# foxcroftjn/polars-strsim

Measured on AMD Instinct MI355X. Metric: M string-pairs/s, levenshtein, 100 M rows (+ achieved HBM GB/s in roofline), higher is better.
Workload: dtype u8/u32 bit-parallel, f64 epilogue

## Files before the change

polars-strsim_amd/csrc/strsim_kernels.hip:

```cpp
#include <hip/hip_runtime.h>
#include <stddef.h>
#include <cstdlib>
#include <stdint.h>
#include <type_traits>

#include "strsim_bounds.h"
#include "strsim_lane_core.h"
#include "strsim_lane_lut.h"
#include "strsim_lane_wide.h"
#include "strsim_lane_sym.h"
#include "strsim_kernels.h"
#include "strsim_lane_common.h"
#include "strsim_osa.h"
#include "strsim_distance.h"
#include "strsim_indel.h"
#include "strsim_partial.h"
#include "strsim_qgram.h"
#include "strsim_token.h"
#include "strsim_wratio.h"
#include "strsim_process.h"
#include "strsim_nearest.h"
#include "strsim_extract.h"
#include "strsim_cdist.h"
#include "strsim_join.h"
#include "strsim_match_join.h"
#include "strsim_components.h"

namespace strsim {

constexpr int ALL_MEASURES = 5;

struct OutPtrs {
    double *p[5];
};

#include "strsim_lane_stage.h"
#if defined(STRSIM_LAB) && defined(STRSIM_STAGE_PC)
#include "strsim_lane_stage_pc.h"
#endif
#include "strsim_lane_lit.h"
#include "strsim_match.h"
#include "strsim_nearest_kernels.h"
#include "strsim_extract_kernels.h"
#include "strsim_cdist_kernels.h"
#include "strsim_join_kernels.h"
#include "strsim_match_join_kernels.h"
#include "strsim_components_kernels.h"

#include "strsim_kernel_wide.h"
#include "strsim_kernel_utf8.h"
#include "strsim_kernel_wave.h"
#include "strsim_kernel_huge.h"

static void wide_geometry(const LaunchArgs &a, int span, uint32_t &sps, unsigned &grid)
{
    const uint64_t nchunks = (a.n + 63u) >> 6;
    const uint64_t nspans = (nchunks + (uint64_t)span - 1) / (uint64_t)span;
    const uint64_t want = 2u * (uint64_t)a.wide_grid;
    uint64_t k = nspans / (want ? want : 1u);
    if (k < 1u) k = 1u;
    if (k > (uint64_t)(WIDE_BLOCK / span)) k = WIDE_BLOCK / span;
    sps = (uint32_t)k;
    const uint64_t nsuper = (nspans + k - 1u) / k;
    grid = (unsigned)(nsuper < (uint64_t)a.wide_grid_cap ? nsuper : (uint64_t)a.wide_grid_cap);
}

static uint64_t stage_launch_size(uint64_t nsb, uint64_t resident, uint64_t cus)
{
    constexpr uint64_t per = 4;
    uint64_t g = nsb / per;
    const uint64_t floor_ = nsb < cus ? nsb : cus;
    if (g < floor_) g = floor_;
    if (g > resident) g = resident;
    return g ? g : 1u;
}

template <int M>
static void launch_lane_t(const LaunchArgs &a)
{
#if defined(STRSIM_LAB) && defined(STRSIM_STAGE_STRIP)
    if (M == LEVENSHTEIN && a.rowsA != 1 && a.rowsB != 1) {
        static uint16_t *buf = nullptr;
        static uint64_t cap = 0;
        if (a.n > cap) { if (buf) (void)hipFree(buf); (void)hipMalloc((void **)&buf, a.n * 2 + 64); cap = a.n; }
        hipLaunchKernelGGL(k_strip_oracle, dim3((unsigned)((a.n + 255) / 256)), dim3(256), 0, a.stream, a.offA, a.valA, a.offB, a.valB, a.n, buf);
        (void)hipMemcpyToSymbolAsync(HIP_SYMBOL(g_strip_ptr), &buf, sizeof buf, 0, hipMemcpyHostToDevice, a.stream);
    }
#endif
    if (a.ev_lane0) (void)hipEventRecord(a.ev_lane0, a.stream);
    OutPtrs op{};
    op.p[0] = a.out;
    const bool lit_a = a.rowsA == 1 && a.rowsB != 1, lit_b = a.rowsB == 1 && a.rowsA != 1;
    const bool lit_path = lit_a || lit_b;
    if (lit_path && !a.no_literal_path) {
        const bool litA = lit_a;
        const uint64_t nlb = (a.n + (LIT_ROWS - 1)) / LIT_ROWS;
        const uint64_t want = (uint64_t)a.stage_grid * 3u;
        const uint64_t gl = nlb < want ? nlb : want;
        hipLaunchKernelGGL((k_lane_lit<M>), dim3((unsigned)gl), dim3(LIT_BLOCK), 0, a.stream, litA ? a.offB : a.offA,
                           litA ? a.valB : a.valA, litA ? a.offA : a.offB, litA ? a.valA : a.valB, a.out, a.n, a.slowmask,
                           a.status, a.qtab, a.sched);
        if (a.publish_host) hipLaunchKernelGGL(k_publish_lit, dim3(1), dim3(64), 0, a.stream, a.sched, a.publish_host, a.publish_ticket);
    } else {
        const uint64_t nsb = (a.n + (STAGE_ROWS - 1)) / STAGE_ROWS;
        auto go = [&](auto tables, auto long_rows) {
            constexpr bool T = decltype(tables)::value, L = decltype(long_rows)::value;
            const uint64_t res = (uint64_t)a.stage_grid * (uint64_t)stage_waves_per_eu<M, T, L>() / (uint64_t)STRSIM_STAGE_WAVES_PER_EU;
            const uint64_t gs = stage_launch_size(nsb, res, (uint64_t)a.stage_grid / (uint64_t)STRSIM_STAGE_WAVES_PER_EU);
            hipLaunchKernelGGL((k_lane_stage<M, T, L>), dim3((unsigned)gs), dim3(STAGE_BLOCK), 0, a.stream, a.offA, a.valA, a.rowsA,
                               a.offB, a.valB, a.rowsB, op, a.n, a.slowmask, a.status, a.qtab, a.sched, a.publish_host, a.publish_ticket);
        };
#if defined(STRSIM_LAB) && defined(STRSIM_STAGE_PC)
        if (((STRSIM_STAGE_PC >> M) & 1) != 0 && a.rowsA != 1 && a.rowsB != 1 && !a.long_rows) {
            const uint64_t cus = (uint64_t)a.stage_grid / (uint64_t)STRSIM_STAGE_WAVES_PER_EU;
            const uint64_t gs = stage_launch_size(nsb, cus * (uint64_t)STRSIM_PC_WG_PER_CU, cus);
            hipLaunchKernelGGL((k_lane_stage_pc<M, STRSIM_PC_LUT != 0>), dim3((unsigned)gs), dim3(PC_THREADS), 0, a.stream, a.offA, a.valA, a.rowsA,
                               a.offB, a.valB, a.rowsB, op, a.n, a.slowmask, a.status, a.qtab, a.sched, a.publish_host, a.publish_ticket);
        } else
#endif
        if (a.long_rows) go(std::false_type{}, std::true_type{});
        else if constexpr (stage_uses_lut<M>()) go(std::true_type{}, std::false_type{});
        else go(std::false_type{}, std::false_type{});
    }
    if (a.ev_lane1) (void)hipEventRecord(a.ev_lane1, a.stream);
}

template <int M>
static void launch_slow_t(const LaunchArgs &a)
{
    const uint64_t nchunks = (a.n + 63u) >> 6;
    const uint64_t wg = M == LEVENSHTEIN ? (uint64_t)a.wave_grid_lev
                        : (M == JARO || M == JARO_WINKLER) ? (uint64_t)a.wave_grid * 3u / 4u : (uint64_t)a.wave_grid;
    const uint64_t g2 = nchunks < wg ? nchunks : wg;
    {
        uint32_t sps, sps8;
        unsigned g3, g8;
        wide_geometry(a, WIDE_SPAN, sps, g3);
        wide_geometry(a, U8_SPAN, sps8, g8);
        hipLaunchKernelGGL((k_lane_wide<M>), dim3(g3), dim3(WIDE_BLOCK), 0, a.stream, a.offA, a.valA, a.rowsA,
                           a.offB, a.valB, a.rowsB, a.out, a.n, a.slowmask, sps);
        hipLaunchKernelGGL((k_lane_utf8<M>), dim3(g8), dim3(WIDE_BLOCK), 0, a.stream, a.offA, a.valA, a.rowsA,
                           a.offB, a.valB, a.rowsB, a.out, a.n, a.slowmask, sps8, a.worklist, a.status);
    }
    hipLaunchKernelGGL((k_wave_pairs<M>), dim3((unsigned)g2), dim3(64), 0, a.stream, a.offA, a.valA, a.rowsA, a.offB,
                       a.valB, a.rowsB, a.out, a.n, a.slowmask, a.worklist, a.status, a.lev_ws);
    if (a.ev_wave1) (void)hipEventRecord(a.ev_wave1, a.stream);
}


template <int M>
static void launch_pair(const LaunchArgs &a)
{
    launch_lane_t<M>(a);
    launch_slow_t<M>(a);
}

template <int M>
static void launch_huge_t(const LaunchArgs &a, uint32_t *ws, uint32_t cap, int grid)
{
    hipLaunchKernelGGL((k_huge_pairs<M>), dim3((unsigned)grid), dim3(64), 0, a.stream, a.offA, a.valA, a.rowsA, a.offB,
                       a.valB, a.rowsB, a.out, a.n, ws, cap);
// ... 702 lines not shown
```

polars-strsim_amd/csrc/strsim_lane_stage.h:

```cpp
#pragma once

#ifndef STRSIM_STAGE_ROWS
#define STRSIM_STAGE_ROWS 512
#endif
#ifndef STRSIM_STAGE_CAP
#define STRSIM_STAGE_CAP 10240
#endif
#ifndef STRSIM_STAGE_CAP_LONG
#define STRSIM_STAGE_CAP_LONG 15104
#endif
#ifndef STRSIM_STAGE_CAP_LUT
#define STRSIM_STAGE_CAP_LUT 8960
#endif
#ifndef STRSIM_STAGE_WAVES_PER_EU
#define STRSIM_STAGE_WAVES_PER_EU 5
#endif
#ifndef STRSIM_STAGE_BUCKET_SHIFT
#define STRSIM_STAGE_BUCKET_SHIFT 1
#endif

#ifndef STRSIM_STAGE_LUT
#define STRSIM_STAGE_LUT 0x26
#endif
#ifndef STRSIM_JARO_KEEP_EQ_FILLS
#define STRSIM_JARO_KEEP_EQ_FILLS 1
#endif
#ifndef STRSIM_STAGE_LONG_TEXT_MAX
#define STRSIM_STAGE_LONG_TEXT_MAX 32
#endif
#ifndef STRSIM_STAGE_RANGE_MAX
#define STRSIM_STAGE_RANGE_MAX 64
#endif
#ifndef STRSIM_STAGE_RANGE_DIV
#define STRSIM_STAGE_RANGE_DIV 4
#endif
#ifndef STRSIM_STAGE_RANGE_MIN_BLOCKS
#define STRSIM_STAGE_RANGE_MIN_BLOCKS 2
#endif

#if defined(STRSIM_LAB) && defined(STRSIM_STAGE_STAMPS)
__device__ unsigned long long g_stage_stamps[16384][16];
#define STAGE_STAMP(cat) do { __builtin_amdgcn_sched_barrier(0); const unsigned long long t_ = __builtin_amdgcn_s_memtime(); \
                              __builtin_amdgcn_sched_barrier(0); st_acc[cat] += t_ - st_last; st_last = t_; } while (0)
#else
#define STAGE_STAMP(cat) do { } while (0)
#endif

#ifndef STRSIM_STAGE_THREADS
#define STRSIM_STAGE_THREADS 256
#endif
constexpr int STAGE_BLOCK = STRSIM_STAGE_THREADS;
constexpr int STAGE_WAVES = STAGE_BLOCK / 64;
constexpr int STAGE_ROWS = STRSIM_STAGE_ROWS;
constexpr int STAGE_RPT = STAGE_ROWS / STAGE_BLOCK;
constexpr int STAGE_NR = STAGE_ROWS / 64;
constexpr int STAGE_RPW = STAGE_NR / STAGE_WAVES;
template <int MEASURE> constexpr bool stage_uses_lut() { return ((STRSIM_STAGE_LUT >> MEASURE) & 1) != 0; }

template <bool TABLES, bool LONG = false> struct StageGeom {
    static_assert(!(TABLES && LONG), "the long-row geometry has no match-mask tables");
    static constexpr int CAP = LONG ? STRSIM_STAGE_CAP_LONG : (TABLES ? STRSIM_STAGE_CAP_LUT : STRSIM_STAGE_CAP);
    static constexpr int COL = CAP + 96;
    static constexpr int DMA_ITERS = (CAP + 48 + 16 * STAGE_BLOCK - 1) / (16 * STAGE_BLOCK);
    static_assert(CAP % 16 == 0 && 2 * COL + 64 + 16 <= 65536, "staging area: whole wave-instructions, 16-bit LDS offsets");
};
constexpr int STAGE_BSH = STRSIM_STAGE_BUCKET_SHIFT;
constexpr int STAGE_NBK = (32 >> STAGE_BSH) + 1;
static_assert(STAGE_RPT >= 1 && STAGE_RPT <= 4 && STAGE_RPW >= 1, "STAGE_ROWS is 256, 512 or 1024");
static_assert(STAGE_NBK <= 32, "the bucket scan runs on 32 lanes");

#define STRSIM_LDS_ADDR(p) ((uint32_t)(uintptr_t)((__attribute__((address_space(3))) void *)(p)))

__device__ __forceinline__ void lds_dma_b128(const void *gbase, uint32_t goff, uint32_t lds_dst)
{
    uint32_t keep;
    asm volatile("s_mov_b32 %0, m0\n\ts_mov_b32 m0, %3\n\ts_nop 0\n\tglobal_load_lds_dwordx4 %1, %2\n\ts_mov_b32 m0, %0"
                 : "=&s"(keep)
                 : "v"(goff), "s"(gbase), "s"(lds_dst)
                 : "memory");
}
__device__ __forceinline__ void lds_dma_b32(const void *gbase, uint32_t goff, uint32_t lds_dst)
{
    uint32_t keep;
    asm volatile("s_mov_b32 %0, m0\n\ts_mov_b32 m0, %3\n\ts_nop 0\n\tglobal_load_lds_dword %1, %2\n\ts_mov_b32 m0, %0"
                 : "=&s"(keep)
                 : "v"(goff), "s"(gbase), "s"(lds_dst)
                 : "memory");
}

__device__ __forceinline__ uint32_t load_invariant(const uint32_t *p)
{
    return *reinterpret_cast<const __attribute__((address_space(4))) uint32_t *>(reinterpret_cast<uintptr_t>(p));
}

constexpr uint32_t STAGE_DEAD = 1u << 31;

#if defined(STRSIM_LAB) && defined(STRSIM_STAGE_STRIP)
__device__ const uint16_t *g_strip_ptr;
__global__ __launch_bounds__(256) void k_strip_oracle(const uint32_t *__restrict__ offA, const uint8_t *__restrict__ valA, const uint32_t *__restrict__ offB,
                                                      const uint8_t *__restrict__ valB, uint64_t n, uint16_t *__restrict__ out)
{
    const uint64_t r = (uint64_t)blockIdx.x * 256u + threadIdx.x;
    if (r >= n) return;
    const uint32_t a0 = offA[r], la = offA[r + 1] - a0, b0 = offB[r], lb = offB[r + 1] - b0;
    const uint32_t m = la < lb ? la : lb, cap = (uint32_t)STRSIM_STAGE_STRIP;
    uint32_t p = 0, s = 0;
    while (p < m && p < cap && valA[a0 + p] == valB[b0 + p]) ++p;
    while (s < m - p && s < cap && valA[a0 + la - 1u - s] == valB[b0 + lb - 1u - s]) ++s;
    if (p + s > 63u) s = 63u - p;
    out[r] = (uint16_t)(p | (s << 8));
}
#define STRSIM_STRIP_ON 1
#else
#define STRSIM_STRIP_ON 0
#endif

__device__ __forceinline__ void stage_window(const uint8_t *base, uint32_t at, uint32_t (&w)[8], uint32_t lds_bytes = 0u, uint32_t who = 0u)
{
    typedef uint32_t u32x4_a4 __attribute__((ext_vector_type(4), aligned(4)));
    (void)lds_bytes; (void)who;
    if (who == 1u) STRSIM_CHECK_RANGE(K_STAGE, 40, ~0ull, (at & ~3u) + 36u, 0, lds_bytes);
    if (who == 2u) STRSIM_CHECK_RANGE(K_LIT, 40, ~0ull, (at & ~3u) + 36u, 0, lds_bytes);
    const uint8_t *q = base + (at & ~3u);
    const u32x4_a4 lo = *reinterpret_cast<const u32x4_a4 *>(q);
    const u32x4_a4 hi = *reinterpret_cast<const u32x4_a4 *>(q + 16);
    const uint32_t top = *reinterpret_cast<const uint32_t *>(q + 32);
    const uint32_t sh = at & 3u;
    w[0] = __builtin_amdgcn_alignbyte(lo.y, lo.x, sh); w[1] = __builtin_amdgcn_alignbyte(lo.z, lo.y, sh);
    w[2] = __builtin_amdgcn_alignbyte(lo.w, lo.z, sh); w[3] = __builtin_amdgcn_alignbyte(hi.x, lo.w, sh);
    w[4] = __builtin_amdgcn_alignbyte(hi.y, hi.x, sh); w[5] = __builtin_amdgcn_alignbyte(hi.z, hi.y, sh);
    w[6] = __builtin_amdgcn_alignbyte(hi.w, hi.z, sh); w[7] = __builtin_amdgcn_alignbyte(top, hi.w, sh);
}

__device__ __forceinline__ uint32_t scan32_inclusive(uint32_t x)
{
    x += (uint32_t)__builtin_amdgcn_update_dpp(0, (int)x, 0x111, 0xF, 0xF, true);
    x += (uint32_t)__builtin_amdgcn_update_dpp(0, (int)x, 0x112, 0xF, 0xF, true);
    x += (uint32_t)__builtin_amdgcn_update_dpp(0, (int)x, 0x114, 0xF, 0xF, true);
    x += (uint32_t)__builtin_amdgcn_update_dpp(0, (int)x, 0x118, 0xF, 0xF, true);
    x += (uint32_t)__builtin_amdgcn_update_dpp(0, (int)x, 0x142, 0xA, 0xF, true);
    return x;
}

template <int NP, bool USE_LUT>
__device__ __forceinline__ uint32_t stage_lev_code(const EqLut &lut, const uint32_t (&wa)[8], uint32_t la, const uint32_t (&wb)[8],
                                                   uint32_t lb, uint32_t tmin, uint32_t tmax, uint32_t stripped = 0u)
{
    uint32_t P[NP];
    build_planes<NP>(wb, P);
    EqLut t = lut;
    if (USE_LUT) lut_build<NP>(t, P, 0xFFFFFFFFu);
    const bool live = la != 0u && lb != 0u;
    const uint32_t la1 = live ? la : 1u, lb1 = live ? lb : 1u;
    const uint32_t dist = USE_LUT ? lev_myers32_lut<NP>(t, wa, la1, tmin, tmax, P, lb1) : lev_myers32_snap<NP>(wa, la1, tmin, tmax, P, lb1);
    uint32_t code = dist * (uint32_t)QTAB_N + (la1 > lb1 ? la1 : lb1);
    if (!live) code = (la == 0u && lb == 0u) ? 1u : (uint32_t)QTAB_N + 1u;
#if STRSIM_STRIP_ON
    const uint32_t longer = la > lb ? la : lb;
    code = (live ? dist : longer) * (uint32_t)QTAB_N + (longer + stripped);
#endif
    return code;
}

template <int NP, bool USE_LUT>
__device__ __forceinline__ unsigned long long stage_all_ints(const EqLut &lut, const uint32_t (&wa)[8], uint32_t la,
                                                             const uint32_t (&wb)[8], uint32_t lb, uint32_t tmin, uint32_t tmax)
{
    uint32_t P[NP];
    build_planes<NP>(wb, P);
    const bool live = la != 0u && lb != 0u;
    const uint32_t la1 = live ? la : 1u, lb1 = live ? lb : 1u;
    uint32_t dist, m, t, isect;
    if (USE_LUT) {
        EqLut tb = lut;
        lut_build<NP>(tb, P, 0xFFFFFFFFu);
        lane_cores32_lut<NP, true, true, true>(tb, wa, la1, tmin, tmax, lb1, P, dist, m, t, isect);
    } else {
        lane_cores32<NP, true, true, true>(wa, la1, tmin, tmax, lb1, P, dist, m, t, isect);
    }
    const uint32_t pre = common_prefix4(wa[0], la1, wb[0], lb1);
    const uint32_t lo = dist | (m << 6) | (t << 12) | (isect << 18) | (pre << 24) | (la << 27);
    return (unsigned long long)lo | ((unsigned long long)(la >> 5) << 32) | ((unsigned long long)lb << 33);
}

__device__ __forceinline__ void stage_all_epilogues(unsigned long long pk, double qa, double qb, double qc, double qd, double (&r)[5])
{
    const uint32_t lo = (uint32_t)pk, hi = (uint32_t)(pk >> 32);
    const uint32_t m = (lo >> 6) & 63u, isect = (lo >> 18) & 63u, pre = (lo >> 24) & 7u;
    const uint32_t la = ((lo >> 27) & 31u) | ((hi & 1u) << 5), lb = (hi >> 1) & 63u;
    if (la == 0u || lb == 0u) {
        const double v = (la == 0u && lb == 0u) ? 1.0 : 0.0;
#pragma unroll
        for (int q = 0; q < 5; ++q) r[q] = v;
        return;
    }
    r[LEVENSHTEIN] = 1.0 - qd;
    const double j = m == 0u ? 0.0 : div3_exact(qa + qb + qc);
    r[JARO] = j;
    r[JARO_WINKLER] = epilogue_jaro_winkler(j, pre);
    r[JACCARD] = epilogue_jaccard(isect, la, lb);
    r[SORENSEN_DICE] = epilogue_sorensen_dice(isect, la, lb);
}

template <int MEASURE, int NP, bool USE_LUT>
__device__ __forceinline__ uint32_t stage_ints(const EqLut &lut, const uint32_t (&wa)[8], uint32_t la, const uint32_t (&wb)[8],
                                               uint32_t lb, uint32_t tmin, uint32_t tmax)
{
    uint32_t P[NP];
    build_planes<NP>(wb, P);
    const bool live = la != 0u && lb != 0u;
    const uint32_t la1 = live ? la : 1u, lb1 = live ? lb : 1u;
    uint32_t dist, m, t, isect;
    EqLut tb = lut;
    if (USE_LUT) lut_build<NP>(tb, P, 0xFFFFFFFFu);
    if (MEASURE == JARO || MEASURE == JARO_WINKLER) {
        if (USE_LUT) lane_cores32_lut<NP, false, true, false>(tb, wa, la1, tmin, tmax, lb1, P, dist, m, t, isect);
        else lane_cores32<NP, false, true, false, STRSIM_JARO_KEEP_EQ_FILLS != 0>(wa, la1, tmin, tmax, lb1, P, dist, m, t, isect);
        const uint32_t pre = MEASURE == JARO_WINKLER ? common_prefix4(wa[0], la1, wb[0], lb1) : 0u;
        return m | (t << 6) | (la << 12) | (lb << 18) | (pre << 24);
    }
    if (USE_LUT) lane_cores32_lut<NP, false, false, true>(tb, wa, la1, tmin, tmax, lb1, P, dist, m, t, isect);
    else lane_cores32<NP, false, false, true>(wa, la1, tmin, tmax, lb1, P, dist, m, t, isect);
    return isect | (la << 6) | (lb << 12);
}

template <int MEASURE>
__device__ __forceinline__ double stage_epilogue(uint32_t pk, double qa, double qb, double qc)
{
    if (MEASURE == JARO || MEASURE == JARO_WINKLER) {
        const uint32_t m = pk & 63u, la = (pk >> 12) & 63u, lb = (pk >> 18) & 63u, pre = (pk >> 24) & 7u;
        if (la == 0u || lb == 0u) return (la == 0u && lb == 0u) ? 1.0 : 0.0;
        const double j = m == 0u ? 0.0 : div3_exact(qa + qb + qc);
        return MEASURE == JARO_WINKLER ? epilogue_jaro_winkler(j, pre) : j;
    }
    const uint32_t isect = pk & 63u, la = (pk >> 6) & 63u, lb = (pk >> 12) & 63u;
    if (la == 0u || lb == 0u) return (la == 0u && lb == 0u) ? 1.0 : 0.0;
    return MEASURE == JACCARD ? epilogue_jaccard(isect, la, lb) : epilogue_sorensen_dice(isect, la, lb);
}

template <int MEASURE, bool LUT>
__device__ __forceinline__ void stage_compute(const EqLut &lut, const uint32_t (&wt)[8], const uint32_t (&wp)[8], uint32_t meta,
                                              uint32_t last, uint16_t *s_code, uint32_t *s_word, double *s_val)
{
    bool fast = (meta & STAGE_DEAD) == 0u;
#if STRSIM_STRIP_ON
    const uint32_t lt = meta & 0x3Fu, lp = (meta >> 8) & 0x3Fu, idx = (meta >> 16) & 0x1FFu, stripped = (meta >> 25) & 0x3Fu;
#else
    const uint32_t lt = meta & 0x3Fu, lp = (meta >> 8) & 0x3Fu, idx = (meta >> 16) & 0x7FFu, stripped = 0u;
#endif
    uint32_t any;
    const uint32_t vary = window_vary(wt, wp, any);
    if (any & 0x80u) fast = false;
    if (__ballot(fast) == 0ull) return;
    const uint32_t la = fast ? lt : 0u, lb = fast ? lp : 0u;
    static_assert((1 << STAGE_BSH) % COLS_PER_TEST == 0, "a bucket's upper bound is a whole number of column groups");
    const uint32_t ltl = (uint32_t)__builtin_amdgcn_readlane((int)lt, (int)last);
    const uint32_t tmax = (((ltl ? ltl : 1u) - 1u) | ((1u << STAGE_BSH) - 1u)) + 1u;
    const bool wide = __ballot(fast && (vary & 0x60u)) != 0ull;
    const uint32_t lt0 = uniform(lt);
    const uint32_t tmin = (((lt0 ? lt0 : 1u) - 1u) & ~((1u << STAGE_BSH) - 1u)) + 1u;
    if (MEASURE == LEVENSHTEIN) {
        uint32_t code;
        if (wide) code = stage_lev_code<7, LUT>(lut, wt, la, wp, lb, tmin, tmax, stripped);
        else code = stage_lev_code<5, LUT>(lut, wt, la, wp, lb, tmin, tmax, stripped);
        if (fast) STRSIM_CHECK_INDEX(K_STAGE, 42, ~0ull, idx, STAGE_ROWS);
        if (fast) s_code[idx] = (uint16_t)code;
    } else if (MEASURE == ALL_MEASURES) {
        unsigned long long pk;
        if (wide) pk = stage_all_ints<7, LUT>(lut, wt, la, wp, lb, tmin, tmax);
        else pk = stage_all_ints<5, LUT>(lut, wt, la, wp, lb, tmin, tmax);
        if (fast) STRSIM_CHECK_INDEX(K_STAGE, 43, ~0ull, idx, STAGE_ROWS);
        if (fast) reinterpret_cast<unsigned long long *>(s_val)[idx] = pk;
    } else {
        uint32_t pk;
        if (wide) pk = stage_ints<MEASURE, 7, LUT>(lut, wt, la, wp, lb, tmin, tmax);
        else pk = stage_ints<MEASURE, 5, LUT>(lut, wt, la, wp, lb, tmin, tmax);
        if (fast) STRSIM_CHECK_INDEX(K_STAGE, 44, ~0ull, idx, STAGE_ROWS);
        if (fast) s_word[idx] = pk;
    }
}

template <int MEASURE, bool LUT, bool LONG = false>
__device__ __forceinline__ void
lane_stage_body(const uint32_t *__restrict__ offA, const uint8_t *__restrict__ valA, uint64_t rowsA,
             const uint32_t *__restrict__ offB, const uint8_t *__restrict__ valB, uint64_t rowsB, OutPtrs outs,
             uint64_t n, unsigned long long *__restrict__ slowmask, DevStatus *__restrict__ status,
             const double *__restrict__ qtab, uint32_t *__restrict__ sched, DevStatus *__restrict__ publish, uint32_t ticket)
{
    constexpr bool LEV = MEASURE == LEVENSHTEIN;
    constexpr bool ALL = MEASURE == ALL_MEASURES;
    constexpr int B = STAGE_ROWS, RPT = STAGE_RPT, NBK = STAGE_NBK;
    constexpr int STAGE_CAP = StageGeom<LUT, LONG>::CAP, STAGE_COL = StageGeom<LUT, LONG>::COL;
    constexpr int STAGE_DMA_ITERS = StageGeom<LUT, LONG>::DMA_ITERS;
    constexpr uint32_t COLB = STAGE_COL, LIT = 2u * STAGE_COL;
    static_assert(!LUT || (B <= 128 * STAGE_WAVES && LUT_WAVE_BYTES == 3072), "descriptor slices: 128 rows behind each wave's tables");
    __shared__ __attribute__((aligned(4096))) uint8_t s_lut[LUT ? 4096 * STAGE_WAVES : 16];
    __shared__ uint2 s_desc_own[LUT ? 1 : B];
    __shared__ __attribute__((aligned(4096))) uint8_t s_bytes[2 * STAGE_COL + 64 + 16];
    auto desc_at = [&](uint32_t p) -> uint2 * {
        if (LUT) return reinterpret_cast<uint2 *>(s_lut + ((p >> 7) << 12) + LUT_WAVE_BYTES + ((p & 127u) << 3));
        return s_desc_own + p;
    };
    __shared__ __attribute__((aligned(16))) uint32_t s_off[2][B + 4];
    __shared__ uint32_t s_cnt[32];
    __shared__ uint32_t s_left;
    __shared__ uint32_t s_sched[2];
    __shared__ uint16_t s_code[LEV ? B : 1];
    __shared__ uint32_t s_word[(!LEV && !ALL) ? B : 1];
    __shared__ double s_val[ALL ? B : 1];

    const uint32_t tid = threadIdx.x, lane = lane_id(), wv = tid >> 6;
    if (blockIdx.x == 0u && tid < (uint32_t)(sizeof(DevStatus) / sizeof(uint32_t))) reinterpret_cast<uint32_t *>(status)[tid] = 0u;
    if (tid < 32u) s_cnt[tid] = 0u;
    if (tid == 0u) s_left = 0u;
#pragma unroll
    for (int q = 0; q < RPT; ++q) {
        const uint32_t i = (uint32_t)q * STAGE_BLOCK + tid;
        if (LEV) s_code[i] = 0xFFFFu;
        else if (ALL) reinterpret_cast<unsigned long long *>(&s_val[i])[0] = ~0ull;
        else s_word[i] = 0xFFFFFFFFu;
    }

    const uint32_t totalA = load_invariant(offA + rowsA), totalB = load_invariant(offB + rowsB);
#if STRSIM_BOUNDS_ON
    const uint32_t firstA = load_invariant(offA), firstB = load_invariant(offB);
#endif
    const bool bcastA = rowsA == 1, bcastB = rowsB == 1;
    const uint32_t litA0 = bcastA ? load_invariant(offA) : 0u, litB0 = bcastB ? load_invariant(offB) : 0u;
    const uint32_t litAlen = bcastA ? totalA - litA0 : 0u, litBlen = bcastB ? totalB - litB0 : 0u;
    if (wv == 0u) {
        auto literal_window = [&](const uint8_t *val, uint32_t at, uint32_t total, uint32_t len, uint32_t *dst) {
            uint32_t w[8];
            load_window32(val, at, total, w);
            const uint32_t rep = (w[0] & 0xFFu) * 0x01010101u;
#pragma unroll
            for (int q = 0; q < 8; ++q) {
                const uint32_t v = len > 4u * q ? (len - 4u * q < 4u ? len - 4u * q : 4u) : 0u;
                const uint32_t keep = v >= 4u ? 0xFFFFFFFFu : ((1u << (8u * v)) - 1u);
                dst[q] = (w[q] & keep) | (rep & ~keep);
            }
        };
        if (bcastA) literal_window(valA, litA0, totalA, litAlen, reinterpret_cast<uint32_t *>(s_bytes + LIT));
        if (bcastB) literal_window(valB, litB0, totalB, litBlen, reinterpret_cast<uint32_t *>(s_bytes + LIT + 32u));
    }
    const uint64_t nchunks = (n + 63u) >> 6;
    const uint32_t nchunks32 = (uint32_t)nchunks;
    auto grab = [&](uint32_t seen, uint32_t &lo, uint32_t &sz) {
        const uint32_t left = nchunks32 > seen ? nchunks32 - seen : 0u;
        uint32_t want = (uint32_t)STRSIM_STAGE_RANGE_MAX;
        if (left < (uint32_t)(STRSIM_STAGE_RANGE_MAX * STRSIM_STAGE_RANGE_DIV) * gridDim.x) want = left / ((uint32_t)STRSIM_STAGE_RANGE_DIV * gridDim.x);
        sz = want < (uint32_t)(STRSIM_STAGE_RANGE_MIN_BLOCKS * (B / 64)) ? (uint32_t)(STRSIM_STAGE_RANGE_MIN_BLOCKS * (B / 64)) : want;
        lo = __hip_atomic_fetch_add(&sched[0], sz, __ATOMIC_RELAXED, __HIP_MEMORY_SCOPE_AGENT);
    };
    uint32_t grab_lo = 0u, grab_sz = 0u;
    if (tid == 0u) {
        grab(0u, grab_lo, grab_sz);
        s_sched[0] = grab_lo;
        s_sched[1] = grab_sz;
    }
    lds_barrier();
    uint64_t row_end;
    uint64_t row0;
    {
        const uint64_t lo = uniform(s_sched[0]), hi = lo + uniform(s_sched[1]);
        row0 = lo * 64u < n ? lo * 64u : n;
        row_end = hi * 64u < n ? hi * 64u : n;
    }
    lds_barrier();
    if (tid == 0u) grab(grab_lo, grab_lo, grab_sz);
    bool grab_pending = true;

    EqLut lut;
    lut.lane4 = lane * 4u;
    lut.krep = ((STRSIM_LDS_ADDR(&s_lut[0]) >> 8) + 16u * wv) * 0x01010101u;
    const uint32_t ldsOffA = STRSIM_LDS_ADDR(&s_off[0][0]), ldsOffB = STRSIM_LDS_ADDR(&s_off[1][0]);
    const uint32_t ldsBytes = STRSIM_LDS_ADDR(&s_bytes[0]);
    const uint32_t wvu = uniform(wv);
    const uint32_t tid4 = tid * 4u, tid16 = tid * 16u;
    auto dma_offsets = [&](uint64_t row) {
        const uint32_t cnt = (uint32_t)(row_end - row < (uint64_t)B ? row_end - row : (uint64_t)B);
        const uint32_t *const pa = offA + row, *const pb = offB + row;
#pragma unroll
        for (int it = 0; it < RPT; ++it) {
            if (tid + (uint32_t)it * STAGE_BLOCK <= cnt) {
                if (!bcastA) STRSIM_CHECK_INDEX(K_STAGE, 1, row, row + (uint64_t)it * STAGE_BLOCK + tid, rowsA + 1u);
                if (!bcastB) STRSIM_CHECK_INDEX(K_STAGE, 2, row, row + (uint64_t)it * STAGE_BLOCK + tid, rowsB + 1u);
                STRSIM_CHECK_INDEX(K_STAGE, 3, row, (uint32_t)it * STAGE_BLOCK + tid, B + 4);
                if (!bcastA) lds_dma_b32(pa + it * STAGE_BLOCK, tid4, ldsOffA + 4u * ((uint32_t)it * STAGE_BLOCK + wvu * 64u));
                if (!bcastB) lds_dma_b32(pb + it * STAGE_BLOCK, tid4, ldsOffB + 4u * ((uint32_t)it * STAGE_BLOCK + wvu * 64u));
            }
        }
        if (tid == 0u && cnt == (uint32_t)B) {
            if (!bcastA) STRSIM_CHECK_INDEX(K_STAGE, 4, row, row + (uint64_t)B, rowsA + 1u);
            if (!bcastB) STRSIM_CHECK_INDEX(K_STAGE, 5, row, row + (uint64_t)B, rowsB + 1u);
            if (!bcastA) lds_dma_b32(pa + B, tid4, ldsOffA + 4u * (uint32_t)B);
            if (!bcastB) lds_dma_b32(pb + B, tid4, ldsOffB + 4u * (uint32_t)B);
        }
    };

    uint64_t prev_row0 = 0;
    uint32_t prev_rows = 0;
    if (row0 < row_end) dma_offsets(row0);
    asm volatile("s_waitcnt vmcnt(0)" ::: "memory");
    lds_barrier();

    auto pin = [](double &x) { asm volatile("" : "+v"(x)); };
    auto store_block = [&](uint64_t r0, uint32_t rows) {
        unsigned long long *__restrict__ const maskb = slowmask + (r0 >> 6);
        constexpr int M1 = (MEASURE == ALL_MEASURES || MEASURE == LEVENSHTEIN) ? JARO : MEASURE;
        constexpr bool JARO_LIKE = ALL || M1 == JARO || M1 == JARO_WINKLER;
        unsigned long long pk[RPT];
        double t0[RPT], t1[RPT], t2[RPT], t3[RPT];
#pragma unroll
        for (int q = 0; q < RPT; ++q) {
            const uint32_t i = (uint32_t)q * STAGE_BLOCK + tid;
            if (ALL) {
                pk[q] = reinterpret_cast<const unsigned long long *>(s_val)[i];
// ... 71 lines not shown
    };

#if defined(STRSIM_LAB) && defined(STRSIM_STAGE_STAMPS)
    unsigned long long st_acc[10] = {0, 0, 0, 0, 0, 0, 0, 0, 0, 0};
    const unsigned long long st_t0 = __builtin_amdgcn_s_memtime(), st_r0 = __builtin_amdgcn_s_memrealtime();
    unsigned long long st_last = st_t0;
#endif
    while (row0 < row_end) {
        if (grab_pending) {
            if (tid == 0u) {
                s_sched[0] = grab_lo;
                s_sched[1] = grab_sz;
            }
            grab_pending = false;
        }
        if (prev_rows) store_block(prev_row0, prev_rows);
        STAGE_STAMP(1);
        const uint32_t avail = (uint32_t)(row_end - row0 < (uint64_t)B ? row_end - row0 : (uint64_t)B);
        const uint32_t baseA = bcastA ? litA0 : uniform(s_off[0][0]), baseB = bcastB ? litB0 : uniform(s_off[1][0]);
        const uint32_t misA = (uint32_t)(reinterpret_cast<uintptr_t>(valA + baseA) & 15u);
        const uint32_t misB = (uint32_t)(reinterpret_cast<uintptr_t>(valB + baseB) & 15u);
        uint32_t rows;
        {
            const uint32_t e = (lane + 1u) * 64u < avail ? (lane + 1u) * 64u : avail;
            const bool exists = lane * 64u < avail && lane < (uint32_t)(B / 64);
            const uint32_t endA = bcastA ? baseA : s_off[0][exists ? e : 0u], endB = bcastB ? baseB : s_off[1][exists ? e : 0u];
            const bool fits = exists && endA - baseA + misA <= (uint32_t)STAGE_CAP && endB - baseB + misB <= (uint32_t)STAGE_CAP;
            const unsigned long long okm = __ballot(fits);
            uint32_t k = (uint32_t)__builtin_ctzll(~okm);
            if (k == 0u) k = 1u;
            rows = uniform(k * 64u < avail ? k * 64u : avail);
        }
        const uint32_t endA = bcastA ? baseA : uniform(s_off[0][rows]), endB = bcastB ? baseB : uniform(s_off[1][rows]);
        const uint32_t spanA = endA - baseA + misA, spanB = endB - baseB + misB;
        const uint32_t stagedA = bcastA ? 0u : (((spanA < (uint32_t)STAGE_CAP ? spanA : (uint32_t)STAGE_CAP) + 15u) & ~15u);
        const uint32_t stagedB = bcastB ? 0u : (((spanB < (uint32_t)STAGE_CAP ? spanB : (uint32_t)STAGE_CAP) + 15u) & ~15u);
        const uint32_t leftA = totalA - baseA + misA, leftB = totalB - baseB + misB;
        const uint32_t chunksA = bcastA ? 0u : ((stagedA + 32u < leftA ? stagedA + 32u : leftA) + 15u) >> 4;
        const uint32_t chunksB = bcastB ? 0u : ((stagedB + 32u < leftB ? stagedB + 32u : leftB) + 15u) >> 4;
        if (tid < 2u) STRSIM_CHECK_RANGE(K_STAGE, 20, row0, (chunksA << 4) + tid * 16u + 16u, 0, COLB);
        else if (tid < 4u) STRSIM_CHECK_RANGE(K_STAGE, 21, row0, COLB + (chunksB << 4) + (tid - 2u) * 16u + 16u, 0, sizeof(s_bytes));
        if (tid < 2u) *reinterpret_cast<uint4 *>(s_bytes + (chunksA << 4) + tid * 16u) = make_uint4(0u, 0u, 0u, 0u);
        else if (tid < 4u) *reinterpret_cast<uint4 *>(s_bytes + COLB + (chunksB << 4) + (tid - 2u) * 16u) = make_uint4(0u, 0u, 0u, 0u);
        {
            const uint8_t *__restrict__ const gA = valA + baseA - misA, *__restrict__ const gB = valB + baseB - misB;
#pragma unroll
            for (int it = 0; it < STAGE_DMA_ITERS; ++it) {
                if (tid + (uint32_t)it * STAGE_BLOCK < chunksA) {
                    STRSIM_CHECK_COLUMN(K_STAGE, 22, row0, gA + 16 * it * STAGE_BLOCK + tid16, 16, valA, firstA, totalA);
                    STRSIM_CHECK_RANGE(K_STAGE, 23, row0, 16u * ((uint32_t)it * STAGE_BLOCK + tid) + 16u, 0, COLB);
                    lds_dma_b128(gA + 16 * it * STAGE_BLOCK, tid16, ldsBytes + 16u * ((uint32_t)it * STAGE_BLOCK + wvu * 64u));
                }
                if (tid + (uint32_t)it * STAGE_BLOCK < chunksB) {
                    STRSIM_CHECK_COLUMN(K_STAGE, 24, row0, gB + 16 * it * STAGE_BLOCK + tid16, 16, valB, firstB, totalB);
                    STRSIM_CHECK_RANGE(K_STAGE, 25, row0, COLB + 16u * ((uint32_t)it * STAGE_BLOCK + tid) + 16u, 0, sizeof(s_bytes));
                    lds_dma_b128(gB + 16 * it * STAGE_BLOCK, tid16, ldsBytes + COLB + 16u * ((uint32_t)it * STAGE_BLOCK + wvu * 64u));
                }
            }
        }
        STAGE_STAMP(0);
        uint32_t skey[RPT], srank[RPT], sd0[RPT], sd1[RPT];
        {
#pragma unroll
            for (int q = 0; q < RPT; ++q) {
                const uint32_t i = (uint32_t)RPT * tid + (uint32_t)q;
                STRSIM_CHECK_INDEX(K_STAGE, 30, row0, i + 1u, B + 4);
                const bool have = i < rows;
                const uint32_t a0 = bcastA ? 0u : s_off[0][i] - baseA, b0 = bcastB ? 0u : s_off[1][i] - baseB;
                const uint32_t la8 = bcastA ? litAlen : s_off[0][i + 1u] - s_off[0][i];
                const uint32_t lb8 = bcastB ? litBlen : s_off[1][i + 1u] - s_off[1][i];
                const bool stA = bcastA || misA + a0 + la8 <= stagedA, stB = bcastB || misB + b0 + lb8 <= stagedB;
                bool mine = have && la8 <= 32u && lb8 <= 32u && stA && stB;
                if (LONG && STRSIM_STAGE_LONG_TEXT_MAX < 32 && !bcastA && !bcastB) mine = mine && (la8 < lb8 ? la8 : lb8) <= (uint32_t)STRSIM_STAGE_LONG_TEXT_MAX;
                const uint32_t wa = bcastA ? LIT : misA + a0, wb = bcastB ? LIT + 32u : COLB + misB + b0;
                const bool swap = !bcastA && !bcastB && la8 > lb8;
#if STRSIM_STRIP_ON
                uint32_t sp = 0u, ss = 0u;
                if (LEV && !bcastA && !bcastB && have) {
                    const uint32_t ps = g_strip_ptr[row0 + i];
                    sp = ps & 0xFFu; ss = ps >> 8;
                }
                const uint32_t lt = (swap ? lb8 : la8) - sp - ss, lp = (swap ? la8 : lb8) - sp - ss;
                const uint32_t key = mine ? (((lt ? lt : 1u) - 1u) >> STAGE_BSH) : (uint32_t)(NBK - 1);
                skey[q] = key;
                srank[q] = atomicAdd(&s_cnt[key], 1u);
                sd0[q] = mine ? (swap ? ((wb + sp) | ((wa + sp) << 16)) : ((wa + sp) | ((wb + sp) << 16))) : 0u;
                sd1[q] = mine ? (lt | (lp << 8) | (i << 16) | ((sp + ss) << 25)) : STAGE_DEAD;
#else
                const uint32_t lt = swap ? lb8 : la8, lp = swap ? la8 : lb8;
                const uint32_t key = mine ? (((lt ? lt : 1u) - 1u) >> STAGE_BSH) : (uint32_t)(NBK - 1);
                skey[q] = key;
                srank[q] = atomicAdd(&s_cnt[key], 1u);
                sd0[q] = mine ? (swap ? (wb | (wa << 16)) : (wa | (wb << 16))) : 0u;
                sd1[q] = mine ? (lt | (lp << 8) | (i << 16)) : STAGE_DEAD;
#endif
            }
        }
        STAGE_STAMP(2);
        lds_barrier();
        STAGE_STAMP(3);
        uint32_t nmine;
        {
            const uint32_t c = s_cnt[lane & 31u];
            const uint32_t exc = scan32_inclusive(c) - c;
#pragma unroll
            for (int q = 0; q < RPT; ++q) {
                const uint32_t base = __shfl(exc, skey[q], 32);
                const uint32_t p = base + srank[q];
                STRSIM_CHECK_INDEX(K_STAGE, 31, row0, p, B);
                *desc_at(p) = make_uint2(sd0[q], sd1[q]);
            }
            nmine = uniform(__shfl(exc, NBK - 1, 32));
        }
        STAGE_STAMP(4);
        asm volatile("s_waitcnt vmcnt(0)" ::: "memory");
        if (!bcastA && leftA < (chunksA << 4) && tid == ((chunksA - 1u) & (uint32_t)(STAGE_BLOCK - 1)))
            for (uint32_t b = leftA; b < (chunksA << 4); ++b) { STRSIM_CHECK_INDEX(K_STAGE, 32, row0, b, COLB); s_bytes[b] = 0; }
        if (!bcastB && leftB < (chunksB << 4) && tid == ((chunksB - 1u) & (uint32_t)(STAGE_BLOCK - 1)))
            for (uint32_t b = leftB; b < (chunksB << 4); ++b) { STRSIM_CHECK_INDEX(K_STAGE, 33, row0, COLB + b, sizeof(s_bytes)); s_bytes[COLB + b] = 0; }
        lds_barrier();
        STAGE_STAMP(5);
        if (tid < 32u) s_cnt[tid] = 0u;
        uint64_t next_row0 = row0 + rows;
        if (next_row0 >= row_end) {
            const uint64_t lo = uniform(s_sched[0]), hi = lo + uniform(s_sched[1]);
            next_row0 = lo * 64u < n ? lo * 64u : n;
            row_end = hi * 64u < n ? hi * 64u : n;
            if (tid == 0u) grab((uint32_t)lo, grab_lo, grab_sz);
            grab_pending = true;
        }
        if (next_row0 < row_end) dma_offsets(next_row0);
        STAGE_STAMP(6);
        __builtin_amdgcn_s_setprio(0);
        {
            const uint32_t nrounds = (nmine + 63u) >> 6;
#pragma unroll 1
            for (int k = 0; k < STAGE_RPW; ++k) {
                const uint32_t t = (uint32_t)(k >> 1) * (2u * STAGE_WAVES) + ((k & 1) ? (uint32_t)(2 * STAGE_WAVES - 1) - wv : wv);
                if (t >= nrounds) continue;
                const uint32_t hi = nmine - 64u * t;
                const uint32_t first = hi >= 64u ? hi - 64u : 0u;
                const uint32_t in_round = hi - first;
                __builtin_amdgcn_s_setprio(1);
                STRSIM_CHECK_INDEX(K_STAGE, 41, row0, first + lane, B);
                const uint2 d = *desc_at(first + lane);
                uint32_t wt[8], wp[8];
                stage_window(s_bytes, d.x & 0xFFFFu, wt, (uint32_t)sizeof(s_bytes), STRSIM_BOUNDS_ON ? 1u : 0u);
                stage_window(s_bytes, d.x >> 16, wp, (uint32_t)sizeof(s_bytes), STRSIM_BOUNDS_ON ? 1u : 0u);
    #if defined(STRSIM_LAB) && defined(STRSIM_STAGE_STAMPS)
                asm volatile("s_waitcnt lgkmcnt(0)" ::: "memory");
    #endif
                STAGE_STAMP(7);
                __builtin_amdgcn_s_setprio(0);
                stage_compute<MEASURE, LUT>(lut, wt, wp, lane < in_round ? d.y : STAGE_DEAD, in_round - 1u, s_code, s_word, s_val);
                STAGE_STAMP(8);
            }
        }
        __builtin_amdgcn_s_setprio(1);
        asm volatile("s_waitcnt vmcnt(0)" ::: "memory");
        lds_barrier();
        STAGE_STAMP(9);
        prev_row0 = row0;
        prev_rows = rows;
        row0 = next_row0;
    }
    if (prev_rows) store_block(prev_row0, prev_rows);
    if (publish) lds_barrier();
    if (tid == 0u) {
        if (publish && s_left) __hip_atomic_fetch_add(&sched[2], s_left, __ATOMIC_RELAXED, __HIP_MEMORY_SCOPE_AGENT);
        const uint32_t done = __hip_atomic_fetch_add(&sched[1], 1u, __ATOMIC_ACQ_REL, __HIP_MEMORY_SCOPE_AGENT);
        if (done == gridDim.x - 1u) {
            if (publish) {
                const uint32_t total = __hip_atomic_load(&sched[2], __ATOMIC_RELAXED, __HIP_MEMORY_SCOPE_AGENT);
                __hip_atomic_store(&publish->lane_left, total, __ATOMIC_RELEASE, __HIP_MEMORY_SCOPE_SYSTEM);
                if (ticket) __hip_atomic_store(&publish->ticket, ticket, __ATOMIC_RELEASE, __HIP_MEMORY_SCOPE_SYSTEM);
            }
            __hip_atomic_store(&sched[0], 0u, __ATOMIC_RELAXED, __HIP_MEMORY_SCOPE_AGENT);
            __hip_atomic_store(&sched[1], 0u, __ATOMIC_RELAXED, __HIP_MEMORY_SCOPE_AGENT);
            __hip_atomic_store(&sched[2], 0u, __ATOMIC_RELAXED, __HIP_MEMORY_SCOPE_AGENT);
        }
    }
#if defined(STRSIM_LAB) && defined(STRSIM_STAGE_STAMPS)
    if (lane == 0u) {
        const uint32_t w = (blockIdx.x * STAGE_WAVES + wv) & 16383u;
        for (int q = 0; q < 10; ++q) g_stage_stamps[w][q] = st_acc[q];
        g_stage_stamps[w][10] = __builtin_amdgcn_s_memtime() - st_t0;
        const unsigned long long st_r1 = __builtin_amdgcn_s_memrealtime();
        g_stage_stamps[w][11] = st_r1 - st_r0;
        g_stage_stamps[w][12] = st_r0;
        g_stage_stamps[w][13] = st_r1;
        g_stage_stamps[w][14] = (unsigned long long)__builtin_amdgcn_s_getreg((4 << 0) | (0 << 6) | (31 << 11));
        g_stage_stamps[w][15] = (unsigned long long)__builtin_amdgcn_s_getreg((20 << 0) | (0 << 6) | (31 << 11));
    }
#endif
}

#ifndef STRSIM_STAGE_PLAIN_WAVES
#define STRSIM_STAGE_PLAIN_WAVES 5
#endif
#ifndef STRSIM_STAGE_ALL_WAVES_PER_EU
#define STRSIM_STAGE_ALL_WAVES_PER_EU 3
#endif
template <int MEASURE, bool TABLES, bool LONG = false> constexpr int stage_waves_per_eu()
{
    constexpr int lim = MEASURE == ALL_MEASURES ? STRSIM_STAGE_ALL_WAVES_PER_EU : ((TABLES || LONG) ? 4 : STRSIM_STAGE_PLAIN_WAVES);
    return STRSIM_STAGE_WAVES_PER_EU < lim ? STRSIM_STAGE_WAVES_PER_EU : lim;
}

template <int MEASURE, bool TABLES, bool LONG = false>
__global__ __launch_bounds__(STAGE_BLOCK) __attribute__((amdgpu_waves_per_eu(stage_waves_per_eu<MEASURE, TABLES, LONG>()))) void
k_lane_stage(const uint32_t *__restrict__ offA, const uint8_t *__restrict__ valA, uint64_t rowsA,
             const uint32_t *__restrict__ offB, const uint8_t *__restrict__ valB, uint64_t rowsB, OutPtrs outs, uint64_t n,
             unsigned long long *__restrict__ slowmask, DevStatus *__restrict__ status, const double *__restrict__ qtab,
             uint32_t *__restrict__ sched, DevStatus *__restrict__ publish, uint32_t ticket)
{
    lane_stage_body<MEASURE, TABLES, LONG>(offA, valA, rowsA, offB, valB, rowsB, outs, n, slowmask, status, qtab, sched, publish, ticket);
}

__global__ __launch_bounds__(STAGE_BLOCK) __attribute__((amdgpu_waves_per_eu(stage_waves_per_eu<ALL_MEASURES, stage_uses_lut<ALL_MEASURES>()>()))) void
k_lane_stage_all(const uint32_t *__restrict__ offA, const uint8_t *__restrict__ valA, uint64_t rowsA,
                 const uint32_t *__restrict__ offB, const uint8_t *__restrict__ valB, uint64_t rowsB, OutPtrs outs, uint64_t n,
                 unsigned long long *__restrict__ slowmask, DevStatus *__restrict__ status, const double *__restrict__ qtab,
                 uint32_t *__restrict__ sched, DevStatus *__restrict__ publish, uint32_t ticket)
{
    lane_stage_body<ALL_MEASURES, stage_uses_lut<ALL_MEASURES>()>(offA, valA, rowsA, offB, valB, rowsB, outs, n, slowmask, status, qtab, sched, publish, ticket);
}
```

Before: 69440.

## Add register permute-table Eq mask builder for 5-plane Levenshtein Myers core

Adds a new Myers bit-parallel core that builds per-character equality masks with a 3+2-bit minterm table held in registers. Lookups go through byte permutes and 4x4 byte transposes instead of per-column bit-plane fills. The stage kernel uses it for narrow (5-plane), non-LUT, non-long Levenshtein buckets once tmax reaches a threshold, and falls back to the existing snap core below it. The aim is to cut per-column ALU work at the cost of a table build per pair plus extra registers. A microbenchmark comparing the two cores is included.

```diff
diff --git a/bench_support/micro/core_ptab.hip b/bench_support/micro/core_ptab.hip
--- /dev/null
+++ b/bench_support/micro/core_ptab.hip
@@ -0,0 +1,87 @@
+#include <hip/hip_runtime.h>
+#include <cstdio>
+#include <cstdint>
+#include "strsim_lane_ptab.h"
+
+template <int CORE>
+__global__ __launch_bounds__(64) void k(uint32_t *out, unsigned long long *clk, uint32_t seed, int iters, uint32_t cols)
+{
+    using namespace strsim;
+    uint32_t wa[8], wb[8];
+#pragma unroll
+    for (int d = 0; d < 8; ++d) {
+        wa[d] = (seed * (2 * d + 3) + threadIdx.x * 0x01010101u) & 0x1F1F1F1Fu;
+        wb[d] = (seed * (2 * d + 5) + threadIdx.x * 0x01000193u) & 0x1F1F1F1Fu;
+    }
+    const uint32_t tmax = wave_uniform(cols), tmin = tmax - 3u, lt = tmin + (threadIdx.x & 3u);
+    const unsigned long long t0 = __builtin_amdgcn_s_memtime(), r0 = __builtin_amdgcn_s_memrealtime();
+    uint32_t acc = 0;
+#pragma unroll 1
+    for (int i = 0; i < iters; ++i) {
+        uint32_t P[5];
+        build_planes<5>(wb, P);
+        const uint32_t dist = CORE == 1 ? lev_myers32_snap<5>(wa, lt, tmin, tmax, P, 32u) : lev_myers32_ptab<5>(wa, lt, tmin, tmax, P, 32u);
+        acc += dist;
+        wa[0] ^= dist & 0x1Fu;
+        wb[7] = (wb[7] + dist) & 0x1F1F1F1Fu;
+    }
+    const unsigned long long t1 = __builtin_amdgcn_s_memtime(), r1 = __builtin_amdgcn_s_memrealtime();
+    out[blockIdx.x * 64 + threadIdx.x] = acc;
+    if (threadIdx.x == 0) { clk[2 * blockIdx.x] = t1 - t0; clk[2 * blockIdx.x + 1] = r1 - r0; }
+}
+
+template <int CORE>
+static double run(int cus, int w, uint32_t cols, uint32_t *first)
+{
+    const int blocks = cus * 4 * w;
+    uint32_t *d;
+    unsigned long long *c;
+    (void)hipMalloc(&d, (size_t)blocks * 64 * 4);
+    (void)hipMalloc(&c, (size_t)blocks * 16);
+    const int iters = 4000;
+    hipLaunchKernelGGL(k<CORE>, dim3(blocks), dim3(64), 0, 0, d, c, 12345u, 200, cols);
+    (void)hipDeviceSynchronize();
+    hipEvent_t a, b;
+    (void)hipEventCreate(&a); (void)hipEventCreate(&b);
+    (void)hipEventRecord(a);
+    hipLaunchKernelGGL(k<CORE>, dim3(blocks), dim3(64), 0, 0, d, c, 12345u, iters, cols);
+    (void)hipEventRecord(b);
+    (void)hipEventSynchronize(b);
+    float ms = 0;
+    (void)hipEventElapsedTime(&ms, a, b);
+    unsigned long long *h = new unsigned long long[2 * blocks];
+    (void)hipMemcpy(h, c, (size_t)blocks * 16, hipMemcpyDeviceToHost);
+    uint32_t ho[64];
+    (void)hipMemcpy(ho, d, sizeof ho, hipMemcpyDeviceToHost);
+    uint32_t sum = 0;
+    for (int i = 0; i < 64; ++i) sum = sum * 31u + ho[i];
+    *first = sum;
+    double cyc = 0, rt = 0;
+    for (int i = 0; i < blocks; ++i) { cyc += (double)h[2 * i]; rt += (double)h[2 * i + 1]; }
+    cyc /= blocks; rt /= blocks;
+    const double ghz = cyc / rt * 0.1;
+    const double per_iter = ms * 1e-3 * ghz * 1e9 / ((double)iters * w);
+    printf("core %s columns=%2u waves/SIMD=%d: %.3f ms, clock %.2f GHz, %.0f cycles of SIMD time per iteration (64 pairs)\n",
+           CORE == 1 ? "bit-fill" : "ptab    ", cols, w, ms, ghz, per_iter);
+    delete[] h;
+    (void)hipEventDestroy(a); (void)hipEventDestroy(b);
+    (void)hipFree(d); (void)hipFree(c);
+    return per_iter;
+}
+
+int main()
+{
+    hipDeviceProp_t p;
+    if (hipGetDeviceProperties(&p, 0) != hipSuccess) { printf("no device\n"); return 1; }
+    const int cus = p.multiProcessorCount;
+    int differ = 0;
+    for (int w : {4, 5})
+        for (uint32_t cols : {8u, 12u, 16u, 32u}) {
+            uint32_t s1, s2;
+            const double c1 = run<1>(cus, w, cols, &s1);
+            const double c2 = run<2>(cus, w, cols, &s2);
+            printf("   results %s (%08x %08x), ptab / bit-fill = %.3f\n", s1 == s2 ? "agree" : "DIFFER", s1, s2, c2 / c1);
+            differ += s1 != s2;
+        }
+    return differ ? 2 : 0;
+}
diff --git a/polars-strsim_amd/csrc/strsim_kernels.hip b/polars-strsim_amd/csrc/strsim_kernels.hip
--- a/polars-strsim_amd/csrc/strsim_kernels.hip
+++ b/polars-strsim_amd/csrc/strsim_kernels.hip
@@ -7,6 +7,7 @@
 #include "strsim_bounds.h"
 #include "strsim_lane_core.h"
 #include "strsim_lane_lut.h"
+#include "strsim_lane_ptab.h"
 #include "strsim_lane_wide.h"
 #include "strsim_lane_sym.h"
 #include "strsim_kernels.h"
diff --git a/polars-strsim_amd/csrc/strsim_lane_ptab.h b/polars-strsim_amd/csrc/strsim_lane_ptab.h
--- /dev/null
+++ b/polars-strsim_amd/csrc/strsim_lane_ptab.h
@@ -0,0 +1,84 @@
+#pragma once
+#include "strsim_lane_core.h"
+
+namespace strsim {
+
+struct PermTab {
+    uint32_t lo[4], hi[4], m[4];
+};
+
+STRSIM_HD void transpose4x4_bytes(uint32_t w0, uint32_t w1, uint32_t w2, uint32_t w3, uint32_t (&r)[4])
+{
+    const uint32_t t0 = perm_b32(w2, w0, 0x05010400u);
+    const uint32_t t1 = perm_b32(w2, w0, 0x07030602u);
+    const uint32_t t2 = perm_b32(w3, w1, 0x05010400u);
+    const uint32_t t3 = perm_b32(w3, w1, 0x07030602u);
+    r[0] = perm_b32(t2, t0, 0x05010400u);
+    r[1] = perm_b32(t2, t0, 0x07030602u);
+    r[2] = perm_b32(t3, t1, 0x05010400u);
+    r[3] = perm_b32(t3, t1, 0x07030602u);
+}
+
+template <int E>
+STRSIM_HD uint32_t ptab_minterm(uint32_t a, uint32_t b, uint32_t c)
+{
+    return bitop3<1 << ((E & 1) * 4 + ((E >> 1) & 1) * 2 + ((E >> 2) & 1))>(a, b, c);
+}
+
+STRSIM_HD void ptab_build(const uint32_t (&P)[5], PermTab &T)
+{
+    transpose4x4_bytes(ptab_minterm<0>(P[0], P[1], P[2]), ptab_minterm<1>(P[0], P[1], P[2]), ptab_minterm<2>(P[0], P[1], P[2]),
+                       ptab_minterm<3>(P[0], P[1], P[2]), T.lo);
+    transpose4x4_bytes(ptab_minterm<4>(P[0], P[1], P[2]), ptab_minterm<5>(P[0], P[1], P[2]), ptab_minterm<6>(P[0], P[1], P[2]),
+                       ptab_minterm<7>(P[0], P[1], P[2]), T.hi);
+    transpose4x4_bytes(ptab_minterm<0>(P[3], P[4], P[4]), ptab_minterm<1>(P[3], P[4], P[4]), ptab_minterm<6>(P[3], P[4], P[4]),
+                       ptab_minterm<7>(P[3], P[4], P[4]), T.m);
+}
+
+STRSIM_HD void ptab_masks(const PermTab &T, uint32_t w, uint32_t (&Eq)[4])
+{
+    const uint32_t sel_l = w & 0x07070707u, sel_h = (w >> 3) & 0x03030303u;
+    uint32_t q[4];
+#pragma unroll
+    for (int s = 0; s < 4; ++s) q[s] = perm_b32(T.hi[s], T.lo[s], sel_l) & perm_b32(T.m[s], T.m[s], sel_h);
+    transpose4x4_bytes(q[0], q[1], q[2], q[3], Eq);
+}
+
+template <int NP>
+STRSIM_HD uint32_t lev_myers32_ptab(const uint32_t (&wt)[8], uint32_t lt, uint32_t tmin, uint32_t tmax, const uint32_t (&P)[NP],
+                                    uint32_t lp)
+{
+    static_assert(NP == 5, "the register tables split five bits into 3 + 2");
+    static_assert(4 % COLS_PER_TEST == 0, "a text dword is a whole number of column groups");
+    PermTab T;
+    ptab_build(P, T);
+    uint32_t Pv = 0xFFFFFFFFu, Mv = 0u;
+    uint32_t Eq[4];
+    unrolled_until<0, 32 / COLS_PER_TEST>([&](auto gc) {
+        constexpr int g = decltype(gc)::value;
+        if ((uint32_t)(COLS_PER_TEST * g) >= tmax) return false;
+        if constexpr ((COLS_PER_TEST * g) % 4 == 0) ptab_masks(T, wt[(COLS_PER_TEST * g) >> 2], Eq);
+        auto column = [&](int j) {
+            const uint32_t E = Eq[j & 3];
+            const uint32_t D0 = bitop3<0xBE>((E & Pv) + Pv, Pv, E) | Mv;
+            const uint32_t nHP = bitop3<0x0E>(Mv, D0, Pv);
+            const uint32_t nX = twice(nHP);
+            const uint32_t HN2 = twice(D0 & Pv);
+            Pv = bitop3<0xF2>(HN2, D0, nX);
+            Mv = bitop3<0x50>(D0, D0, nX);
+        };
+        if ((uint32_t)(COLS_PER_TEST * (g + 1)) >= tmin) {
+#pragma unroll
+            for (int jj = 0; jj < COLS_PER_TEST; ++jj)
+                if ((uint32_t)(COLS_PER_TEST * g + jj) < lt) column(COLS_PER_TEST * g + jj);
+        } else {
+#pragma unroll
+            for (int jj = 0; jj < COLS_PER_TEST; ++jj) column(COLS_PER_TEST * g + jj);
+        }
+        return true;
+    });
+    const uint32_t rows = low_ones(lp);
+    return lt + popc32(Pv & rows) - popc32(Mv & rows);
+}
+
+}
diff --git a/polars-strsim_amd/csrc/strsim_lane_stage.h b/polars-strsim_amd/csrc/strsim_lane_stage.h
--- a/polars-strsim_amd/csrc/strsim_lane_stage.h
+++ b/polars-strsim_amd/csrc/strsim_lane_stage.h
@@ -21,6 +21,9 @@
 
 #ifndef STRSIM_STAGE_LUT
 #define STRSIM_STAGE_LUT 0x26
+#endif
+#ifndef STRSIM_STAGE_PTAB_MIN
+#define STRSIM_STAGE_PTAB_MIN 12
 #endif
 #ifndef STRSIM_JARO_KEEP_EQ_FILLS
 #define STRSIM_JARO_KEEP_EQ_FILLS 1
@@ -142,7 +145,7 @@
     return x;
 }
 
-template <int NP, bool USE_LUT>
+template <int NP, bool USE_LUT, bool PTAB = false>
 __device__ __forceinline__ uint32_t stage_lev_code(const EqLut &lut, const uint32_t (&wa)[8], uint32_t la, const uint32_t (&wb)[8],
                                                    uint32_t lb, uint32_t tmin, uint32_t tmax, uint32_t stripped = 0u)
 {
@@ -152,7 +155,13 @@
     if (USE_LUT) lut_build<NP>(t, P, 0xFFFFFFFFu);
     const bool live = la != 0u && lb != 0u;
     const uint32_t la1 = live ? la : 1u, lb1 = live ? lb : 1u;
-    const uint32_t dist = USE_LUT ? lev_myers32_lut<NP>(t, wa, la1, tmin, tmax, P, lb1) : lev_myers32_snap<NP>(wa, la1, tmin, tmax, P, lb1);
+    uint32_t dist;
+    if constexpr (PTAB && NP == 5 && !USE_LUT && STRSIM_STAGE_PTAB_MIN <= 32) {
+        if (tmax >= (uint32_t)STRSIM_STAGE_PTAB_MIN) dist = lev_myers32_ptab<NP>(wa, la1, tmin, tmax, P, lb1);
+        else dist = lev_myers32_snap<NP>(wa, la1, tmin, tmax, P, lb1);
+    } else {
+        dist = USE_LUT ? lev_myers32_lut<NP>(t, wa, la1, tmin, tmax, P, lb1) : lev_myers32_snap<NP>(wa, la1, tmin, tmax, P, lb1);
+    }
     uint32_t code = dist * (uint32_t)QTAB_N + (la1 > lb1 ? la1 : lb1);
     if (!live) code = (la == 0u && lb == 0u) ? 1u : (uint32_t)QTAB_N + 1u;
 #if STRSIM_STRIP_ON
@@ -238,7 +247,7 @@
     return MEASURE == JACCARD ? epilogue_jaccard(isect, la, lb) : epilogue_sorensen_dice(isect, la, lb);
 }
 
-template <int MEASURE, bool LUT>
+template <int MEASURE, bool LUT, bool PTAB = false>
 __device__ __forceinline__ void stage_compute(const EqLut &lut, const uint32_t (&wt)[8], const uint32_t (&wp)[8], uint32_t meta,
                                               uint32_t last, uint16_t *s_code, uint32_t *s_word, double *s_val)
 {
@@ -262,7 +271,7 @@
     if (MEASURE == LEVENSHTEIN) {
         uint32_t code;
         if (wide) code = stage_lev_code<7, LUT>(lut, wt, la, wp, lb, tmin, tmax, stripped);
-        else code = stage_lev_code<5, LUT>(lut, wt, la, wp, lb, tmin, tmax, stripped);
+        else code = stage_lev_code<5, LUT, PTAB>(lut, wt, la, wp, lb, tmin, tmax, stripped);
         if (fast) STRSIM_CHECK_INDEX(K_STAGE, 42, ~0ull, idx, STAGE_ROWS);
         if (fast) s_code[idx] = (uint16_t)code;
     } else if (MEASURE == ALL_MEASURES) {
@@ -640,7 +649,7 @@
     #endif
                 STAGE_STAMP(7);
                 __builtin_amdgcn_s_setprio(0);
-                stage_compute<MEASURE, LUT>(lut, wt, wp, lane < in_round ? d.y : STAGE_DEAD, in_round - 1u, s_code, s_word, s_val);
+                stage_compute<MEASURE, LUT, LEV && !LUT && !LONG>(lut, wt, wp, lane < in_round ? d.y : STAGE_DEAD, in_round - 1u, s_code, s_word, s_val);
                 STAGE_STAMP(8);
             }
         }
```

Measured after the change: 73550, median of 6. +5.9%, better.
